# urbste/OpenImuCameraCalibrator

Measured on AMD Instinct MI355X. Metric: residual+Jacobian blocks/sec; wall-clock per LM iter, GoPro9 full calib, higher is better.
Workload: dtype f64

## Files before the change

### openimucameracalibrator_amd/csrc/kernels_bcr.hip

```cpp
#include <hip/hip_runtime.h>
#include <mutex>
#include <unordered_map>
#include "oicc_device.h"
#include "lm_decide.h"
#include "lm_launch.h"
#include "lm_retract.h"
#include "../../include/oicc_hip.h"

namespace oicc {


struct BcrArgs {
  double* D;
  double* F;
  double* S;
  double* Lf;
  double* Mc;
  double* x;
  int32_t* fail;
  long long* prof;
  int n, a, Pb, rtf, LD;
  int delay;
  int o, s, p, m, pn;
  int64_t offS_in, offS_out;
  int carry;
  int last;
  int side;
  int top_l, top_r;
  int b0, ghost;
  const LmCtl* ctl;
};
#define BCR_RETURN_IF_DONE(A) do { if ((A).ctl != nullptr && (A).ctl->done != 0) return; } while (0)

__device__ __forceinline__ void bcr_lds_barrier() { asm volatile("s_waitcnt lgkmcnt(0)\n\ts_barrier" ::: "memory"); }
__device__ __forceinline__ double bcr_readlane(double v, int lane) {
  const int lo = __builtin_amdgcn_readlane(__double2loint(v), lane);
  const int hi = __builtin_amdgcn_readlane(__double2hiint(v), lane);
  return __hiloint2double(hi, lo);
}
typedef double bcr_v4d __attribute__((ext_vector_type(4)));

__device__ __forceinline__ void tri10(int t, int& xt, int& yt) {
  xt = t < 1 ? 0 : (t < 3 ? 1 : (t < 6 ? 2 : 3));
  yt = t - (xt * (xt + 1)) / 2;
}

template <int LD>
__device__ __forceinline__ void bcr_corner_solve(double* C, double* da, int* failp, int a, int tid, int wave, int lane) {
  const int a1 = a + 1;
  if (a1 <= 16) {
    if (wave == 0) {
      double av[16], dinv = 0.0;
#pragma unroll
      for (int c = 0; c < 16; ++c) av[c] = (c < a && lane < a1 && lane >= c) ? C[c * LD + lane] : 0.0;
      bool bad = false;
#pragma unroll
      for (int c = 0; c < 16; ++c) {
        if (c < a) {
          const double piv = bcr_readlane(av[c], c);
          bad |= !(piv > 0.0);
          const double y0 = __builtin_amdgcn_rsq(piv);
          const double g0 = piv * y0, h0 = 0.5 * y0;
          const double r0 = fma(-g0, h0, 0.5);
// ... 63 lines not shown
constexpr int kBackWaves = 8;
constexpr int kInvWaves = 16;
constexpr int kInvLD = 145;

template <int XT>
__device__ __forceinline__ bcr_v4d bcri_z_tile(const double* W, int yt, int li, int lq) {
  constexpr int LD = kInvLD, K0 = 4 * XT, NK = 16 - K0;
  const double* py = W + lq * LD + 64 + 16 * yt + li;
  const double* px = W + lq * LD + 64 + 16 * XT + li;
  double vy[NK], vx[NK];
#pragma unroll
  for (int kk = 0; kk < NK; ++kk) { vy[kk] = py[4 * (K0 + kk) * LD]; vx[kk] = px[4 * (K0 + kk) * LD]; }
  asm volatile("" ::: "memory");
  bcr_v4d g = {0.0, 0.0, 0.0, 0.0}, g2 = {0.0, 0.0, 0.0, 0.0};
#pragma unroll
  for (int kk = 0; kk < NK; kk += 2) {
    g = __builtin_amdgcn_mfma_f64_16x16x4f64(vy[kk], vx[kk], g, 0, 0, 0);
    g2 = __builtin_amdgcn_mfma_f64_16x16x4f64(vy[kk + 1], vx[kk + 1], g2, 0, 0, 0);
  }
  g += g2;
  return g;
}

template <bool LAST>
__device__ __forceinline__ void bcri_tail(const BcrArgs& A, double* W, double* da, int* failp, const double* Fs, double* Zg, int tid, int wave, int lane, bool report,
                                          const double (&ttop)[16], const double ytop, double* x0s) {
  constexpr int LD = kInvLD, NW = kInvWaves, NT = 64 * NW, FLD = 65;
  const int li = lane & 15, lq = lane >> 4;
  const int a = A.a, a1 = a + 1;
  for (int t = wave; t < 10; t += NW) {
    int xt, yt; tri10(t, xt, yt);
    const bcr_v4d g = xt == 0 ? bcri_z_tile<0>(W, yt, li, lq) : (xt == 1 ? bcri_z_tile<1>(W, yt, li, lq) : (xt == 2 ? bcri_z_tile<2>(W, yt, li, lq) : bcri_z_tile<3>(W, yt, li, lq)));
#pragma unroll
    for (int r = 0; r < 4; ++r) {
      const int x = 16 * xt + li, y = 16 * yt + lq + 4 * r;
      if (LAST) { W[y * LD + x] = g[r]; if (xt != yt) W[x * LD + y] = g[r]; }
      else { Zg[y * 64 + x] = g[r]; if (xt != yt) Zg[x * 64 + y] = g[r]; }
    }
  }
  __syncthreads();
  if (!LAST) {
    if (report && tid == 0 && *failp) atomicOr(A.fail, 1);
    return;
  }
  const int rtf = A.rtf;
  if (wave < 4 * rtf) {
    const int t = wave >> 2, w = wave & 3;
    const double* pf = Fs + lq * FLD + 16 * t + li;
    const double* pz = W + lq * LD + 16 * w + li;
    double vf[16], vz[16];
#pragma unroll
    for (int kk = 0; kk < 16; ++kk) { vf[kk] = pf[4 * kk * FLD]; vz[kk] = pz[4 * kk * LD]; }
    asm volatile("" ::: "memory");
    bcr_v4d tq = {0.0, 0.0, 0.0, 0.0};
#pragma unroll
    for (int kk = 0; kk < 16; ++kk) tq = __builtin_amdgcn_mfma_f64_16x16x4f64(vf[kk], vz[kk], tq, 0, 0, 0);
#pragma unroll
    for (int r = 0; r < 4; ++r) W[(16 * w + li) * LD + 64 + 16 * t + lq + 4 * r] = tq[r];
  }
  __syncthreads();
  if (wave < (rtf * (rtf + 1)) / 2) {
    int t1 = 0, u = wave; while (u >= t1 + 1) { u -= t1 + 1; ++t1; }
    const int t2 = u;
    const double* pt = W + lq * LD + 64 + 16 * t1 + li;
    const double* pf = Fs + lq * FLD + 16 * t2 + li;
    double vt[16], vf[16];
#pragma unroll
    for (int kk = 0; kk < 16; ++kk) { vt[kk] = pt[4 * kk * LD]; vf[kk] = pf[4 * kk * FLD]; }
    asm volatile("" ::: "memory");
    bcr_v4d g = {0.0, 0.0, 0.0, 0.0};
#pragma unroll
    for (int kk = 0; kk < 16; ++kk) g = __builtin_amdgcn_mfma_f64_16x16x4f64(vf[kk], vt[kk], g, 0, 0, 0);
    const double* Sm = A.side != 0 ? A.Lf + (int64_t)A.last * (192 + a1) * 64 + 4096 + 64 * a1 : nullptr;
    double mc[4];
#pragma unroll
    for (int r = 0; r < 4; ++r) { const int q1 = 16 * t1 + li, q2 = 16 * t2 + lq + 4 * r; mc[r] = (q1 < a1 && q2 < a1) ? A.Mc[q1 * a1 + q2] + (Sm != nullptr ? Sm[q1 * a1 + q2] : 0.0) : 0.0; }
#pragma unroll
    for (int r = 0; r < 4; ++r) { const int q1 = 16 * t1 + li, q2 = 16 * t2 + lq + 4 * r; if (q1 < a1 && q2 < a1) W[q2 * LD + q1] = mc[r] - g[r]; }
  }
  __syncthreads();
  bcr_corner_solve<LD>(W, da, failp, a, tid, wave, lane);
  for (int q = tid; q < a; q += NT) A.x[A.Pb + q] = da[q];
  if (wave == 0) {
    const double* tc = W + lane * LD + 64;
    double v = tc[a];
    for (int q = 0; q < a; q += 8) {
      double t8[8], d8[8];
#pragma unroll
      for (int k = 0; k < 8; ++k) { const bool ok = q + k < a; t8[k] = ok ? tc[q + k] : 0.0; d8[k] = ok ? da[q + k] : 0.0; }
#pragma unroll
      for (int k = 0; k < 8; ++k) v = fma(-t8[k], d8[k], v);
    }
    const int gi = A.last * 64 + lane;
    if (gi < A.Pb) A.x[gi] = v;
    x0s[lane] = gi < A.Pb ? v : 0.0;
  }
  __syncthreads();
  if (tid == 0 && *failp) atomicOr(A.fail, 1);
  if (A.top_l >= 0 || A.top_r >= 0) {
    double sum_r = 0.0, sum_l = 0.0;
#pragma unroll
    for (int k = 0; k < 4; ++k) {
      const int r = wave + NW * k;
      const double xn = x0s[r], xa = r < a ? da[r] : 0.0;
      sum_r = fma(ttop[k], xn, sum_r);     sum_r = fma(ttop[4 + k], xa, sum_r);
      sum_l = fma(ttop[8 + k], xn, sum_l); sum_l = fma(ttop[12 + k], xa, sum_l);
    }
    W[wave * 64 + lane] = sum_r;
    W[(NW + wave) * 64 + lane] = sum_l;
    __syncthreads();
    if (wave < 2) {
      const int blk = wave == 0 ? A.top_r : A.top_l;
      double acc = 0.0;
#pragma unroll
      for (int w = 0; w < NW; ++w) acc += W[(wave * NW + w) * 64 + lane];
      const int gi = blk * 64 + lane;
      if (blk >= 0 && gi < A.Pb) A.x[gi] = ytop - acc;
    }
  }
}


template <bool LAST, bool PROF, class LoadD>
__device__ __forceinline__ void bcri_invert_body(const BcrArgs& A, const int i, LoadD load_d, const bool report = true) {
  constexpr int LD = kInvLD, NW = kInvWaves, NT = 64 * NW, NTILE = 20, SLOTS = (NTILE + NW - 1) / NW, RU = 128, NAW = 3, FLD = 65;
  static_assert(NW == 16, "the corner phases of block 0 take one tile per wave");
  extern __shared__ double lds[];
  const int tid = threadIdx.x, lane = tid & 63;
  const int wave = __builtin_amdgcn_readfirstlane(tid >> 6);
  const int li = lane & 15, lq = lane >> 4;
  double* const W = lds;
  double* const da = W + 64 * LD;
  int* const failp = reinterpret_cast<int*>(da + 64);
  double* const dg = da + 64 + 8;
  double* const Fs = dg + 256;
  const int a1 = A.a + 1;
  double* Zg = A.Lf + (int64_t)i * (192 + a1) * 64;
  const double* Fg = A.F + (int64_t)i * 64 * a1;
  const double* Sf = (LAST && A.side != 0) ? Zg + 4096 : nullptr;
  const bool prof = PROF && A.prof != nullptr && blockIdx.x == 0 && wave == 0;
  long long pc[8] = {0, 0, 0, 0, 0, 0, 0, 0};
  long long tprev = prof ? clock64() : 0;
// ... 97 lines not shown
#pragma unroll
      for (int k = 0; k < SLOTS; ++k) {
        if (t_ok[k] && t_ct[k] > p && (t_rt[k] < 4 || t_rt[k] - 4 <= p)) {
          const double* pa = W + (j0 + lq) * LD + 16 * t_ct[k] + li;
          const double* pb = W + (j0 + lq) * LD + 16 * t_rt[k] + li;
          double va[4], vb[4];
#pragma unroll
          for (int kq = 0; kq < 4; ++kq) { va[kq] = pa[4 * kq * LD]; vb[kq] = -pb[4 * kq * LD]; }
#pragma unroll
          for (int kq = 0; kq < 4; ++kq) acc[k] = __builtin_amdgcn_mfma_f64_16x16x4f64(va[kq], vb[kq], acc[k], 0, 0, 0);
          if (t_ct[k] == p + 1) {
            double* dst = W + (16 * t_ct[k] + lq) * LD + 16 * t_rt[k] + li;
            dst[0] = acc[k][0]; dst[4 * LD] = acc[k][1]; dst[8 * LD] = acc[k][2]; dst[12 * LD] = acc[k][3];
            if (t_rt[k] == t_ct[k]) { dg[lq * 16 + li] = acc[k][0]; dg[(lq + 4) * 16 + li] = acc[k][1]; dg[(lq + 8) * 16 + li] = acc[k][2]; dg[(lq + 12) * 16 + li] = acc[k][3]; }
          }
        }
      }
    }
    BCR_MARK(3);
    bcr_lds_barrier();
    BCR_MARK(4);
  }
  BCR_MARK(4);
  bcri_tail<LAST>(A, W, da, failp, Fs, Zg, tid, wave, lane, report, ttop, ytop, dg);
  BCR_MARK(5);
  if (PROF && prof && lane == 0) for (int k = 0; k < 8; ++k) A.prof[k] = pc[k];
#undef BCR_MARK
}

template <bool LAST, bool PROF>
__global__ __launch_bounds__(64 * kInvWaves) void bcri_invert_kernel(BcrArgs A) {
  BCR_RETURN_IF_DONE(A);
  const int i = LAST ? A.last : A.o + A.s * (2 * (int)blockIdx.x + A.p);
  const double* Dg = A.D + (int64_t)i * 4096;
  const double* Sd = (LAST && A.side != 0) ? A.Lf + (int64_t)i * (192 + A.a + 1) * 64 : nullptr;
  bcri_invert_body<LAST, PROF>(A, i, [Dg, Sd](int e) { double v = Dg[e]; if (LAST && Sd != nullptr && (e & 63) >= (e >> 6)) v += Sd[e]; return v; });
}

__global__ __launch_bounds__(256) void bcri_schur_kernel(BcrArgs A) {
  BCR_RETURN_IF_DONE(A);
  __shared__ double Ts[16][68];
  const int tid = threadIdx.x, lane = tid & 63;
  const int wave = __builtin_amdgcn_readfirstlane(tid >> 6);
  const int li = lane & 15, lq = lane >> 4;
  const int a1 = A.a + 1, rtf = A.rtf, s = A.s;
  if ((int)blockIdx.y == (int)gridDim.y - 1 && A.carry > 0) {
    const int m = A.carry;
    const double* src = A.S + (A.offS_in + (m - 1)) * 4096; double* dst = A.S + (A.offS_out + (m - 1) / 2) * 4096;
    for (int e = (int)blockIdx.x * 256 + tid; e < 4096; e += (int)gridDim.x * 256) dst[e] = src[e];
// ... 87 lines not shown
      const int x = 16 * xt + li, y = 16 * yt + lq + 4 * r;
      if (to_side) { if (x >= y) Sd[y * 64 + x] = v; }
      else if (x >= y && v != 0.0) unsafeAtomicAdd((xk == 0 ? Dl : Dr) + y * 64 + x, v);
    } else if (yk < 2) {
      const int q = 16 * xt + li, y = 16 * yt + lq + 4 * r;
      if (to_side) { if (q < a1) Sd[4096 + y * a1 + q] = v; }
      else if (q < a1 && v != 0.0) unsafeAtomicAdd((yk == 0 ? Fl : Fr) + y * a1 + q, v);
    } else {
      const int q1 = 16 * xt + li, q2 = 16 * yt + lq + 4 * r;
      if (to_side) { if (q1 < a1 && q2 <= q1) { Sd[4096 + 64 * a1 + q1 * a1 + q2] = v; Sd[4096 + 64 * a1 + q2 * a1 + q1] = v; } }
      else if (q1 < a1 && q2 <= q1 && v != 0.0) {
        unsafeAtomicAdd(A.Mc + q1 * a1 + q2, v);
        if (q1 != q2) unsafeAtomicAdd(A.Mc + q2 * a1 + q1, v);
      }
    }
  }
}

struct BcrOwn {
  int e = -1, code = -1;
  double sc0 = 0.0, d2 = 0.0, g = 0.0;
  const double* x = nullptr; double* xc = nullptr;
};
constexpr int kRetractPark = 12;
template <int NB>
__device__ __forceinline__ BcrOwn bcr_retract_claim(const BcrArgs& A, const RetractReq& R, const SolveBuffers& sb, int b_lo, int b_hi, bool arrow_wg, int tid) {
  BcrOwn o; o.x = R.x; o.xc = R.xc;
  NormalEq ne = R.ne;
  if (A.ctl != nullptr) { o.x = A.ctl->xp[0]; o.xc = A.ctl->xp[1]; ne.base = A.ctl->nep[0]; }
  const int e_hi = b_hi * 64 < A.Pb ? b_hi * 64 : A.Pb;
  if (tid < 64 * NB) { const int e = b_lo * 64 + tid; if (e < e_hi) o.e = e; }
  else if (tid < 64 * NB + A.a && arrow_wg) o.e = A.Pb + (tid - 64 * NB);
  if (o.e >= 0) { o.code = R.rmap[o.e]; o.sc0 = sb.scale[o.e]; o.d2 = sb.D2[o.e]; o.g = ne.g()[o.e]; }
  return o;
}
__device__ __forceinline__ int bcr_rm_steps(int kind) { return kind == kRmEucl ? 1 : (kind == kRmTic ? 6 : 3); }
__device__ __forceinline__ int bcr_rm_params(int kind) { return kind == kRmEucl ? 1 : (kind == kRmTic ? 7 : (kind == kRmSo3 || kind == kRmPt ? 4 : 3)); }
__device__ __forceinline__ void bcr_retract_park(const SolveBuffers& sb, const BcrOwn& o, double* rpark, int stride, int tid) {
  if (o.code < 0) return;
  const int kind = o.code & 7; const int64_t po = o.code >> 3;
  const int nd = bcr_rm_steps(kind), np = bcr_rm_params(kind);
  for (int c = 0; c < np; ++c) rpark[c * stride + tid] = o.x[po + c];
  for (int c = 1; c < nd; ++c) rpark[(6 + c) * stride + tid] = sb.scale[o.e + c];
}
template <int OW>
__device__ __forceinline__ void bcr_retract_finish(const BcrArgs& A, const RetractReq& R, const SolveBuffers& sb, const BcrOwn& o, const double* xflat, int e_base,
                                                   const double* xarrow, const double* rpark, int stride, double* red, int tid, int wave, int lane) {
  __syncthreads();
  if (blockIdx.x == 0 && tid == 0) {
    if (A.ctl != nullptr) { if (A.ctl->stamps != nullptr && A.ctl->seq < A.ctl->trace_cap) A.ctl->stamps[3 * A.ctl->seq + 1] = wall_clock64(); }
    else *R.ne.cost() = 0.0;
  }
  double step_sq = 0.0, x_sq = 0.0, model = 0.0;
  if (o.e >= 0) {
    auto step_at = [&](int e) { return e >= A.Pb ? xarrow[e - A.Pb] : xflat[e - e_base]; };
    model = lm_model_term(step_at(o.e), o.d2, o.g, o.sc0);
    if (o.code >= 0) {
      const int kind = o.code & 7;
      const double alpha = R.alpha;
      const int nd = bcr_rm_steps(kind), np = bcr_rm_params(kind);
      double d[6], sc[6], pv[7];
#pragma unroll
      for (int c = 0; c < 6; ++c) { d[c] = c < nd ? step_at(o.e + c) : 0.0; sc[c] = c == 0 ? o.sc0 : (c < nd ? rpark[(6 + c) * stride + tid] : 0.0); }
#pragma unroll
      for (int c = 0; c < 7; ++c) pv[c] = c < np ? rpark[c * stride + tid] : 0.0;
      double* out = o.xc + (o.code >> 3);
      if (kind == kRmSo3) lm_store_so3(lm_retract_so3(Quat{pv[0], pv[1], pv[2], pv[3]}, d, sc, alpha), pv, out, step_sq, x_sq);
      else if (kind == kRmEucl) lm_retract_eucl(pv[0], d[0], sc[0], alpha, out, step_sq, x_sq);
      else if (kind == kRmAb || kind == kRmGb) { const double bound = kind == kRmAb ? R.max_ab : R.max_gb; for (int c = 0; c < 3; ++c) lm_retract_box(pv[c], d[c], sc[c], alpha, bound, out + c, step_sq, x_sq); }
      else if (kind == kRmPt) lm_retract_point(pv, d, sc, alpha, out, step_sq, x_sq);
      else if (kind == kRmTic) lm_retract_tic(pv, d, sc, alpha, out, step_sq, x_sq);
    }
  }
  if (wave < OW) {
#pragma unroll
    for (int off = 32; off > 0; off >>= 1) { step_sq += __shfl_xor(step_sq, off); x_sq += __shfl_xor(x_sq, off); model += __shfl_xor(model, off); }
    if (lane == 0) { red[wave] = step_sq; red[64 + wave] = x_sq; red[128 + wave] = model; }
  }
  __syncthreads();
  if (tid < 3) {
    double acc = 0.0;
    for (int w = 0; w < OW; ++w) acc += red[64 * tid + w];
    unsafeAtomicAdd(tid == 0 ? &sb.st->step_norm_sq : (tid == 1 ? &sb.st->x_norm_sq : &sb.st->model_cost_change), acc);
  }
}

__global__ __launch_bounds__(64 * kBackWaves) void bcri_backward_kernel(BcrArgs A) {
  BCR_RETURN_IF_DONE(A);
  __shared__ double xs[192];
  __shared__ double part[kBackWaves][64];
  const int tid = threadIdx.x, lane = tid & 63;
  const int wave = __builtin_amdgcn_readfirstlane(tid >> 6);
  const int a = A.a, a1 = a + 1, s = A.s;
  const int kp = 2 * (int)blockIdx.x + A.p;
  const int i = A.o + kp * s, il = i - s;
  const bool hasL = kp > 0;
  const bool hasR = kp < A.m - 1 || A.ghost != 0;
  const int ir = kp < A.m - 1 ? i + s : A.n;
  const double* Tg = A.Lf + (int64_t)i * (192 + a1) * 64 + 4096;
  constexpr int RW = 192 / kBackWaves;
  double lv[RW];
#pragma unroll
  for (int k = 0; k < RW; ++k) {
    const int r = wave + kBackWaves * k;
    const bool ok = r < 128 + a && (hasL || r >= 64) && (hasR || r < 64 || r >= 128);
    lv[k] = ok ? Tg[r * 64 + lane] : 0.0;
  }
  const double yv = wave == 0 ? Tg[(128 + a) * 64 + lane] : 0.0;
  double xin = 0.0;
  if (tid < 64) { const int gi = il * 64 + tid; xin = (hasL && gi < A.Pb) ? A.x[gi] : 0.0; }
  else if (tid < 128) { const int gi = ir * 64 + (tid - 64); xin = (hasR && gi < A.Pb) ? A.x[gi] : 0.0; }
  else if (tid < 128 + a) xin = A.x[A.Pb + (tid - 128)];
  if (tid < 192) xs[tid] = xin;
  __syncthreads();
  double sum = 0.0;
#pragma unroll
  for (int k = 0; k < RW; ++k) { const int r = wave + kBackWaves * k; sum = fma(lv[k], r < 128 + a ? xs[r] : 0.0, sum); }
  part[wave][lane] = sum;
  __syncthreads();
  if (wave == 0) {
    double acc = 0.0;
#pragma unroll
    for (int w = 0; w < kBackWaves; ++w) acc += part[w][lane];
    const int gi = i * 64 + lane;
    if (gi < A.Pb) A.x[gi] = yv - acc;
  }
}

template <bool RETRACT>
__device__ __forceinline__ void bcri_backward2_body(const BcrArgs& A, int ou, int pu, int mu, int npiv_upper, int orphan_l, int orphan_r, const RetractReq& R, const SolveBuffers& sb) {
  constexpr int NW = 16, RW1 = 192 / NW, RW2 = 192 / (NW / 2);
  __shared__ double xw[6][64];
  __shared__ double part[NW][64];
  double* const xs0 = xw[0]; double* const xs1 = xw[2]; double* const xs2 = xw[4]; double* const xs3 = xw[5];
  const int tid = threadIdx.x, lane = tid & 63;
  const int wave = __builtin_amdgcn_readfirstlane(tid >> 6);
  const int a = A.a, a1 = a + 1, s = A.s, n = A.n;
  const int64_t ru64 = (int64_t)(192 + a1) * 64;
  const int lone_ix = (int)blockIdx.x - npiv_upper;
  const bool lone = lone_ix >= 0;
  const bool lone_l = lone && orphan_l >= 0 && lone_ix == 0, lone_r = lone && !lone_l;
  const int ku = 2 * (int)blockIdx.x + pu;
  const int j = lone_l ? orphan_l - s : (lone_r ? orphan_r + s : ou + ku * 2 * s);
  const int jl = j - 2 * s, jr = j + 2 * s;
  const bool ghost = A.ghost != 0;
  const bool has_jl = lone_r || (!lone && ku > 0);
  const bool has_jr = lone_l || (!lone && (ku < mu - 1 || ghost));
  const int jrs = (!lone && ku == mu - 1) ? n : jr;
  const int half = wave >> 3, hw = wave & 7;
  const int ci = half == 0 ? j - s : j + s;
  const bool child = lone ? (half == 0 ? lone_r : lone_l) : (half == 0 ? ci >= A.o : ci <= A.o + (A.m - 1) * s);
  const bool child_hasL = half == 0 ? has_jl : !lone;
  const bool child_hasR = half == 0 ? (!lone || ghost) : has_jr;
  auto xin = [&](int blk, int r) { const int gi = blk * 64 + r; return gi < A.Pb ? A.x[gi] : 0.0; };
  if (tid < 64) xs0[tid] = has_jl ? xin(jl, tid) : 0.0;
  else if (tid < 128) xs2[tid - 64] = has_jr ? xin(jrs, tid - 64) : 0.0;
  else if (tid < 192) xs3[tid - 128] = tid - 128 < a ? A.x[A.Pb + (tid - 128)] : 0.0;
  else if (tid < 256 && lone) xs1[tid - 192] = (lone_r && ghost) ? xin(n, tid - 192) : 0.0;
  __shared__ double rpark[RETRACT ? kRetractPark : 1][384];
  BcrOwn own;
  if (RETRACT) {
    const int b_lo = j - 2 > 0 ? j - 2 : 0;
    int b_hi = j + 2 < n ? j + 2 : n;
    if (!lone && (int)blockIdx.x == npiv_upper - 1 && orphan_r < 0) b_hi = n;
    own = bcr_retract_claim<5>(A, R, sb, b_lo, b_hi, blockIdx.x == 0, tid);
  }
  double l1[RW1], l2[RW2], y1 = 0.0, y2 = 0.0;
  {
    const double* T1 = A.Lf + (lone ? 0 : j) * ru64 + 4096;
#pragma unroll
    for (int k = 0; k < RW1; ++k) {
      const int r = wave + NW * k;
      const bool ok = !lone && r < 128 + a && (has_jl || r >= 64) && (has_jr || r < 64 || r >= 128);
      l1[k] = ok ? T1[r * 64 + lane] : 0.0;
    }
    if (wave == 0 && !lone) y1 = T1[(128 + a) * 64 + lane];
    const double* T2 = A.Lf + (child ? ci : 0) * ru64 + 4096;
#pragma unroll
    for (int k = 0; k < RW2; ++k) {
      const int r = hw + 8 * k;
      const bool ok = child && r < 128 + a && (child_hasL || r >= 64) && (child_hasR || r < 64 || r >= 128);
      l2[k] = ok ? T2[r * 64 + lane] : 0.0;
    }
    if (hw == 0 && child) y2 = T2[(128 + a) * 64 + lane];
  }
  if (RETRACT) bcr_retract_park(sb, own, &rpark[0][0], 384, tid);
  __syncthreads();
  if (!lone) {
    double sum = 0.0;
#pragma unroll
    for (int k = 0; k < RW1; ++k) {
      const int r = wave + NW * k;
      const double xv = r < 64 ? xs0[r] : (r < 128 ? xs2[r - 64] : (r < 128 + a ? xs3[r - 128] : 0.0));
      sum = fma(l1[k], xv, sum);
    }
    part[wave][lane] = sum;
    __syncthreads();
    if (wave == 0) {
      double acc = 0.0;
#pragma unroll
      for (int w = 0; w < NW; ++w) acc += part[w][lane];
      const double xv = y1 - acc;
      const int gi = j * 64 + lane;
      xs1[lane] = gi < A.Pb ? xv : 0.0;
      if (gi < A.Pb) A.x[gi] = xv;
    }
    __syncthreads();
  }
  {
    const double* xl = half == 0 ? xs0 : xs1;
    const double* xr = half == 0 ? xs1 : xs2;
    double sum = 0.0;
#pragma unroll
    for (int k = 0; k < RW2; ++k) {
      const int r = hw + 8 * k;
      const double xv = r < 64 ? xl[r] : (r < 128 ? xr[r - 64] : (r < 128 + a ? xs3[r - 128] : 0.0));
      sum = fma(l2[k], xv, sum);
    }
    part[wave][lane] = sum;
    __syncthreads();
    if (hw == 0 && child) {
      double acc = 0.0;
#pragma unroll
      for (int w = 0; w < 8; ++w) acc += part[8 * half + w][lane];
      const int gi = ci * 64 + lane;
      const double xv = y2 - acc;
      if (gi < A.Pb) A.x[gi] = xv;
      if (RETRACT) xw[half == 0 ? 1 : 3][lane] = gi < A.Pb ? xv : 0.0;
    }
  }
  if (RETRACT) bcr_retract_finish<6>(A, R, sb, own, &xw[0][0], (j - 2) * 64, xs3, &rpark[0][0], 384, &part[0][0], tid, wave, lane);
}
__global__ __launch_bounds__(1024) void bcri_backward2_kernel(BcrArgs A, int ou, int pu, int mu, int npiv_upper, int orphan_l, int orphan_r) {
  BCR_RETURN_IF_DONE(A);
  bcri_backward2_body<false>(A, ou, pu, mu, npiv_upper, orphan_l, orphan_r, RetractReq{}, SolveBuffers{});
}
__global__ __launch_bounds__(1024) void bcri_backward2_retract_kernel(BcrArgs A, int ou, int pu, int mu, int npiv_upper, int orphan_l, int orphan_r, RetractReq R, SolveBuffers sb) {
  BCR_RETURN_IF_DONE(A);
  bcri_backward2_body<true>(A, ou, pu, mu, npiv_upper, orphan_l, orphan_r, R, sb);
}

__device__ __forceinline__ void bcr_build_body(const NormalEq& ne, const TangentLayout& tl, const SolveBuffers& sb, int reuse_diagonal, double min_diag,
                                               double max_diag, const BcrArgs& A, const int64_t tid, const int64_t nthreads) {
  const int Pb = tl.Pb, a = tl.a, W = tl.W, a1 = a + 1, hb = tl.hb, n = A.n;
  const int64_t r0 = (int64_t)A.b0 * 64;
  const double radius = sb.radius;
  if (tid == 0) {
    sb.st->radius = radius; sb.st->model_cost_change = 0.0; sb.st->step_norm_sq = 0.0; sb.st->x_norm_sq = 0.0; sb.st->cand_cost = 0.0; sb.st->chol_failed = 0;
    if (sb.ctl != nullptr && sb.ctl->stamps != nullptr && sb.ctl->seq < sb.ctl->trace_cap) sb.ctl->stamps[3 * sb.ctl->seq] = wall_clock64();
  }
  auto damp = [&](int64_t i, double hii) -> double {
    const double sc = sb.scale[i];
    return (reuse_diagonal ? sb.diag[i] : fmin(fmax(hii * sc * sc, min_diag), max_diag)) / radius;
  };
  for (int64_t i = tid; i < tl.P; i += nthreads) {
    const double hii = i < Pb ? ne.band()[i * W] : ne.C()[(i - Pb) * a + (i - Pb)];
    const double sc = sb.scale[i];
    double d;
    if (!reuse_diagonal) { d = fmin(fmax(hii * sc * sc, min_diag), max_diag); sb.diag[i] = d; }
    else d = sb.diag[i];
    sb.D2[i] = d / radius;
  }
// ... 162 lines not shown
  const int g = A.ghost != 0 ? 1 : 0;
  for (int l = 0; l < L.nlev; ++l) {
    const int m = L.active[l], npiv = L.npivs[l];
    bcr_set_level(A, L, l);
    A.side = (l == L.nlev - 1 && L.parity[l] == 0) ? 1 : 0;
    const bool carry = g != 0 && (m & 1) != 0;
    A.carry = carry ? m : 0;
    BcrArgs Ai = A; if (l != 0) Ai.prof = nullptr;
    if (!(level0_inverted && l == 0)) hipLaunchKernelGGL(k_inv, dim3(npiv), dim3(64 * kInvWaves), bcr_lds_inv(), st, Ai);
    hipLaunchKernelGGL(bcri_schur_kernel, dim3(12 + 3 * A.rtf, npiv + (carry ? 1 : 0)), dim3(256), 0, st, A);
  }
}
static bool bcr_launch_back(BcrArgs A, const BcrLevels& L, int top, hipStream_t st, const RetractReq* R = nullptr, const SolveBuffers* sb = nullptr) {
  int l = top;
  bool fused = false;
  if (l >= 0 && !(l & 1)) { bcr_set_level(A, L, l); hipLaunchKernelGGL(bcri_backward_kernel, dim3(L.npivs[l]), dim3(64 * kBackWaves), 0, st, A); --l; }
  for (; l >= 1; l -= 2) {
    const int lo = l - 1;
    const int orphan_l = (L.parity[lo] == 0 && L.parity[l] == 1) ? L.origin[lo] : -1;
    const int orphan_r = (((L.active[lo] - 1) & 1) == L.parity[lo] && ((L.active[l] - 1) & 1) != L.parity[l]) ? L.origin[lo] + (L.active[lo] - 1) * L.strides[lo] : -1;
    bcr_set_level(A, L, lo);
    const dim3 grid(L.npivs[l] + (orphan_l >= 0 ? 1 : 0) + (orphan_r >= 0 ? 1 : 0));
    if (lo == 0 && R != nullptr) {
      hipLaunchKernelGGL(bcri_backward2_retract_kernel, grid, dim3(1024), 0, st, A, L.origin[l], L.parity[l], L.active[l], L.npivs[l], orphan_l, orphan_r, *R, *sb);
      fused = true;
    } else hipLaunchKernelGGL(bcri_backward2_kernel, grid, dim3(1024), 0, st, A, L.origin[l], L.parity[l], L.active[l], L.npivs[l], orphan_l, orphan_r);
  }
  return fused;
}
static bool bcr_launch_last_and_back(BcrArgs A, const BcrLevels& L, hipStream_t st, const RetractReq* R = nullptr, const SolveBuffers* sb = nullptr) {
  using KernelFn = void (*)(BcrArgs);
  KernelFn k_inv_last = bcri_invert_kernel<true, false>;
  const size_t lds_inv_last = bcr_lds_inv() + (size_t)64 * 65 * sizeof(double);
  bcr_allow_lds(reinterpret_cast<const void*>(k_inv_last), lds_inv_last);
  const int nlev = L.nlev;
  A.o = 0; A.s = 0; A.p = 1; A.m = 1; A.pn = 1; A.offS_in = 0; A.offS_out = 0; A.carry = 0;
  A.last = L.last; A.top_l = -1; A.top_r = -1; A.side = (nlev >= 1 && L.parity[nlev - 1] == 0) ? 1 : 0;
  if (nlev >= 1) {
    const int t = nlev - 1;
    A.top_r = L.last + L.strides[t];
    if (L.parity[t] == 0) A.top_l = L.last - L.strides[t];
  }
  hipLaunchKernelGGL(k_inv_last, dim3(1), dim3(64 * kInvWaves), lds_inv_last, st, A);
  return bcr_launch_back(A, L, nlev - 2, st, R, sb);
}

int bcr_route(const TangentLayout& tl, const SolveBuffers& sb) {
  if (!bcr_applicable(tl) || tl.a + 1 > sb.bcr_max_border || sb.ws == nullptr || sb.ws_doubles < bcr_workspace_doubles(tl)) return kRouteNone;
  if (sb.algo != 0 && sb.algo != 4) return kRouteNone;
  return bcr_fused_build(bcr_blocks(tl.Pb), sb.prof) ? kRouteBcrFused : kRouteBcrUnfused;
}
int launch_bcr_solve(const NormalEq& ne, const TangentLayout& tl, const SolveBuffers& sb, int reuse_diagonal,
                     double min_diag, double max_diag, hipStream_t st, const RetractReq* retract, bool* fused) {
  if (fused) *fused = false;
  if (bcr_route(tl, sb) == kRouteNone) return -1;
  const int n = bcr_blocks(tl.Pb), a1 = tl.a + 1;
  BcrArgs A{};
  bcr_carve(A, sb.ws, n, a1);
  A.Mc = sb.Mc; A.x = sb.step_s; A.fail = &sb.st->chol_failed; A.prof = sb.prof;
  A.n = n; A.a = tl.a; A.Pb = tl.Pb; A.delay = sb.bcr_delay;
  A.rtf = (a1 + 15) / 16; A.ctl = sb.ctl;
  const BcrLevels L = bcr_plan(n, 0, false);
  const bool inverted = bcr_launch_build(ne, tl, sb, reuse_diagonal, min_diag, max_diag, A, L, st);
  bcr_launch_forward(A, inverted, L, st);
  const bool honour = retract != nullptr && retract->on != 0 && retract->rmap != nullptr && retract->alpha == 1.0 && L.nlev >= 3 && A.ghost == 0 && A.b0 == 0;
  RetractReq R{}; if (honour) { R = *retract; R.ne = ne; }
  const bool did = bcr_launch_last_and_back(A, L, st, honour ? &R : nullptr, &sb);
  if (fused) *fused = did;
  return 0;
}

__global__ void bcr_dist_pack_kernel(BcrArgs A, int64_t off_final, double* msg) {
  const int a1 = A.a + 1; const int64_t fsz = (int64_t)64 * a1;
  const int64_t total = 3 * 4096 + 2 * fsz + (int64_t)a1 * a1;
  for (int64_t e = (int64_t)blockIdx.x * blockDim.x + threadIdx.x; e < total; e += (int64_t)gridDim.x * blockDim.x) {
    double v;
    if (e < 4096) v = A.D[e];
    else if (e < 4096 + fsz) v = A.F[e - 4096];
    else if (e < 2 * 4096 + fsz) v = A.ghost ? A.S[off_final * 4096 + (e - 4096 - fsz)] : 0.0;
    else if (e < 3 * 4096 + fsz) v = A.ghost ? A.D[(int64_t)A.n * 4096 + (e - 2 * 4096 - fsz)] : 0.0;
    else if (e < 3 * 4096 + 2 * fsz) v = A.ghost ? A.F[(int64_t)A.n * fsz + (e - 3 * 4096 - fsz)] : 0.0;
    else v = A.Mc[e - 3 * 4096 - 2 * fsz];
    msg[e] = v;
  }
}
__global__ void bcr_dist_top_kernel(BcrArgs T, const double* msgs, int64_t piece) {
  const int N = T.n, a1 = T.a + 1; const int64_t fsz = (int64_t)64 * a1;
  const int64_t nD = (int64_t)N * 4096, nF = (int64_t)N * fsz, nS = (int64_t)(N - 1) * 4096, nC = (int64_t)a1 * a1;
// ... 113 lines not shown
```

### openimucameracalibrator_amd/csrc/oicc_problem.hip

```cpp
#include "oicc_problem.h"

namespace oicc {

int eval_pass(oicc_problem* p, const PassRequest& rq) {
  const double* const x = rq.x; const bool jac = rq.jac; const int only_kind = rq.only_kind;
  const oicc_allreduce_fn reduce = rq.local ? nullptr : p->reduce;
  hipStream_t st = p->stream;
  const NormalEq ne = rq.target ? *rq.target : p->ne;
  if (p->opt["debug_poison_lds"] != 0.0) launch_lds_poison(st);
  {
    const bool with_points = jac && p->tl.a_pts > 0 && (only_kind < 0 || only_kind == 0);
    if (jac && (p->tp.direct || p->tp.n_tiles == 0)) HIPCK(p, hipMemsetAsync(ne.base, 0, ne.total * sizeof(double), st));
    else if (jac && p->tl.a_pts > 0) {
      const int a_np = p->tl.a - p->tl.a_pts;
      HIPCK(p, hipMemsetAsync(ne.base + ne.off_E + int64_t(a_np) * p->tl.Pb, 0, size_t(ne.off_g - ne.off_E - int64_t(a_np) * p->tl.Pb) * sizeof(double), st));
      HIPCK(p, hipMemsetAsync(ne.g() + p->tl.Pb + a_np, 0, size_t(p->tl.a_pts) * sizeof(double), st));
    }
    else if (!jac && !rq.cost_already_zero) HIPCK(p, hipMemsetAsync(ne.cost(), 0, sizeof(double), st));
    const TileParams& tp = p->tp;
    const bool gmax_folded = jac && rq.gmax_into != nullptr && !tp.direct && tp.n_tiles > 0 && !reduce && p->tl.a_pts == 0;
    if (rq.gmax_folded) *rq.gmax_folded = gmax_folded;
    if (!p->h_tstatic) { p->h_tstatic.reset(new TileStatic); std::memset(p->h_tstatic.get(), 0, sizeof(TileStatic)); p->tstatic_valid = false; }
    {
      static_assert(std::is_trivially_copyable<TileStatic>::value, "TileStatic is copied bytewise");
// ... 892 lines not shown
  float ms = 0; (void)hipEventElapsedTime(&ms, ev.a, ev.b);
  if (ms_per_solve) *ms_per_solve = double(ms) / std::max(repeats, 1);
  return OICC_OK;
}

int oicc_solve_residual(oicc_problem* p, int32_t flags, double radius, double out[3]) {
  int rc = prepare(p, flags); if (rc) return rc;
  SolveBuffers sb = solve_buffers(p);
  rc = system_at_current_point(p, local_pass(p->d_x.p, true), sb.scale, p->opt["jacobi_scaling"] != 0, 0.0); if (rc) return rc;
  if (p->tl.P == 0) { out[0] = out[1] = out[2] = 0.0; return OICC_OK; }
  if (launch_lm_solve(p->ne, p->tl, sb, radius, 0, p->opt["min_lm_diagonal"], p->opt["max_lm_diagonal"], p->stream) != 0) { p->err = "solver geometry unsupported"; return OICC_ERR_UNSUPPORTED; }
  return read_solve_residual(p, sb, &out[0], &out[1], &out[2]);
}



double oicc_debug_ls_next_step_size(const double init[3], const double* prev, int32_t prev_has_slope, const double cur[3], int32_t cur_has_slope) {
  LsSample i, q, c;
  i.x = init[0]; i.value = init[1]; i.gradient = init[2]; i.has_gradient = true;
  c.x = cur[0]; c.value = cur[1]; c.gradient = cur[2]; c.has_gradient = cur_has_slope != 0;
  if (prev) { q.x = prev[0]; q.value = prev[1]; q.gradient = prev[2]; q.has_gradient = prev_has_slope != 0; }
  return ls_next_step_size(i, prev ? &q : nullptr, c);
}
int oicc_debug_solver_profile(oicc_problem* p, int32_t flags, long long out[12]) {
  int rc = prepare(p, flags); if (rc) return rc;
  hipStream_t st = p->stream;
  const TangentLayout& tl = p->tl;
  DevBuf<long long> d; if (!d.resize(12)) return OICC_ERR_HIP;
  SolveBuffers sb = solve_buffers(p, d.p);
  rc = system_at_current_point(p, full_system_pass(p), sb.scale, true, 1e4); if (rc) return rc;
  for (int rep = 0; rep < 2; ++rep) {
    if (launch_lm_solve(p->ne, tl, sb, 1e4, 0, 1e-6, 1e32, st) != 0) return OICC_ERR_UNSUPPORTED;
  }
  HIPCK(p, hipMemcpyAsync(out, d.p, 12 * sizeof(long long), hipMemcpyDeviceToHost, st));
  HIPCK(p, hipStreamSynchronize(st));
  return OICC_OK;
}

static int tile_profile(oicc_problem* p, int32_t flags, int32_t kind, long long* out, int n_out) {
  int rc = prepare(p, flags); if (rc) return rc;
  DevBuf<long long> d; if (!d.resize(16)) return OICC_ERR_HIP;
  HIPCK(p, hipMemsetAsync(d.p, 0, 16 * sizeof(long long), p->stream));
  PassRequest rq = local_pass(p->d_x.p, true, kind); rq.prof = d.p;
  rc = eval_pass(p, rq); if (rc) return rc;
  HIPCK(p, hipMemcpyAsync(out, d.p, size_t(n_out) * sizeof(long long), hipMemcpyDeviceToHost, p->stream));
  HIPCK(p, hipStreamSynchronize(p->stream));
  return OICC_OK;
}
int oicc_debug_tile_profile(oicc_problem* p, int32_t flags, int32_t kind, long long out[16]) { return tile_profile(p, flags, kind, out, 16); }
int oicc_debug_block_profile(oicc_problem* p, int32_t flags, int32_t kind, long long out[4]) { return tile_profile(p, flags, kind % 10, out, 4); }
int oicc_debug_view_profile(oicc_problem* p, int32_t flags, long long out[4]) { return oicc_debug_block_profile(p, flags, 0, out); }

int oicc_get_T_i_c(const oicc_problem* p, double v[7]) { std::memcpy(v, p->x.data() + p->pl.tic, 7 * sizeof(double)); return OICC_OK; }
int oicc_get_gravity(const oicc_problem* p, double g[3]) { std::memcpy(g, p->x.data() + p->pl.g, 3 * sizeof(double)); return OICC_OK; }
int oicc_get_rs_line_delay(const oicc_problem* p, double* s) { *s = p->x[p->pl.ld]; return OICC_OK; }
int oicc_get_imu_intrinsics(const oicc_problem* p, double a[6], double g[9]) {
  std::memcpy(a, p->x.data() + p->pl.ai, 6 * sizeof(double)); std::memcpy(g, p->x.data() + p->pl.gi, 9 * sizeof(double)); return OICC_OK; }
int64_t oicc_get_num_accl_bias_knots(const oicc_problem* p) { return p->pl.n_ab; }
int64_t oicc_get_num_gyro_bias_knots(const oicc_problem* p) { return p->pl.n_gb; }
int oicc_get_bias_knots(const oicc_problem* p, double* a, int64_t na, double* g, int64_t ng) {
// ... 60 lines not shown
```

Before: 50.75 million.

## Move arrow retraction into a dedicated block and prefetch retract parameters early

The fused backward-substitution and retraction kernel now gives the arrow (global parameter) retraction its own extra workgroup. Before, those threads were claimed inside block 0's retraction, so that block carried the extra work. Retraction parameter loads are issued into registers before the first barrier and written to LDS after the partial sums, shrinking the LDS park buffer from 12 to 6 rows and overlapping global loads with compute. The fused path is skipped when the tic block lives in the block-tridiagonal part. Profiling timers are also added to the last inversion tail, plus a new debug entry point.

```diff
diff --git a/openimucameracalibrator_amd/csrc/kernels_bcr.hip b/openimucameracalibrator_amd/csrc/kernels_bcr.hip
--- a/openimucameracalibrator_amd/csrc/kernels_bcr.hip
+++ b/openimucameracalibrator_amd/csrc/kernels_bcr.hip
@@ -39,6 +39,8 @@
   return __hiloint2double(hi, lo);
 }
 typedef double bcr_v4d __attribute__((ext_vector_type(4)));
+typedef const __attribute__((address_space(1))) double* bcr_gptr;
+__device__ __forceinline__ bcr_gptr bcr_global(const double* p) { return (bcr_gptr)p; }
 
 __device__ __forceinline__ void tri10(int t, int& xt, int& yt) {
   xt = t < 1 ? 0 : (t < 3 ? 1 : (t < 6 ? 2 : 3));
@@ -148,12 +150,14 @@
   return g;
 }
 
-template <bool LAST>
+template <bool LAST, bool PROF>
 __device__ __forceinline__ void bcri_tail(const BcrArgs& A, double* W, double* da, int* failp, const double* Fs, double* Zg, int tid, int wave, int lane, bool report,
-                                          const double (&ttop)[16], const double ytop, double* x0s) {
+                                          const double (&ttop)[16], const double ytop, double* x0s, const bool prof) {
   constexpr int LD = kInvLD, NW = kInvWaves, NT = 64 * NW, FLD = 65;
   const int li = lane & 15, lq = lane >> 4;
   const int a = A.a, a1 = a + 1;
+  long long tprev = (PROF && prof) ? clock64() : 0;
+#define BCR_TMARK(k) do { if (PROF && prof) { const long long tn_ = clock64(); if (lane == 0) A.prof[20 + (k)] = tn_ - tprev; tprev = tn_; } } while (0)
   for (int t = wave; t < 10; t += NW) {
     int xt, yt; tri10(t, xt, yt);
     const bcr_v4d g = xt == 0 ? bcri_z_tile<0>(W, yt, li, lq) : (xt == 1 ? bcri_z_tile<1>(W, yt, li, lq) : (xt == 2 ? bcri_z_tile<2>(W, yt, li, lq) : bcri_z_tile<3>(W, yt, li, lq)));
@@ -165,6 +169,7 @@
     }
   }
   __syncthreads();
+  BCR_TMARK(0);
   if (!LAST) {
     if (report && tid == 0 && *failp) atomicOr(A.fail, 1);
     return;
@@ -185,6 +190,7 @@
     for (int r = 0; r < 4; ++r) W[(16 * w + li) * LD + 64 + 16 * t + lq + 4 * r] = tq[r];
   }
   __syncthreads();
+  BCR_TMARK(1);
   if (wave < (rtf * (rtf + 1)) / 2) {
     int t1 = 0, u = wave; while (u >= t1 + 1) { u -= t1 + 1; ++t1; }
     const int t2 = u;
@@ -205,7 +211,9 @@
     for (int r = 0; r < 4; ++r) { const int q1 = 16 * t1 + li, q2 = 16 * t2 + lq + 4 * r; if (q1 < a1 && q2 < a1) W[q2 * LD + q1] = mc[r] - g[r]; }
   }
   __syncthreads();
+  BCR_TMARK(2);
   bcr_corner_solve<LD>(W, da, failp, a, tid, wave, lane);
+  BCR_TMARK(3);
   for (int q = tid; q < a; q += NT) A.x[A.Pb + q] = da[q];
   if (wave == 0) {
     const double* tc = W + lane * LD + 64;
@@ -222,6 +230,7 @@
     x0s[lane] = gi < A.Pb ? v : 0.0;
   }
   __syncthreads();
+  BCR_TMARK(4);
   if (tid == 0 && *failp) atomicOr(A.fail, 1);
   if (A.top_l >= 0 || A.top_r >= 0) {
     double sum_r = 0.0, sum_l = 0.0;
@@ -244,6 +253,8 @@
       if (blk >= 0 && gi < A.Pb) A.x[gi] = ytop - acc;
     }
   }
+  BCR_TMARK(5);
+#undef BCR_TMARK
 }
 
 
@@ -387,9 +398,9 @@
     BCR_MARK(4);
   }
   BCR_MARK(4);
-  bcri_tail<LAST>(A, W, da, failp, Fs, Zg, tid, wave, lane, report, ttop, ytop, dg);
+  bcri_tail<LAST, PROF>(A, W, da, failp, Fs, Zg, tid, wave, lane, report, ttop, ytop, dg, prof);
   BCR_MARK(5);
-  if (PROF && prof && lane == 0) for (int k = 0; k < 8; ++k) A.prof[k] = pc[k];
+  if (PROF && prof && lane == 0) for (int k = 0; k < 8; ++k) A.prof[(LAST ? 12 : 0) + k] = pc[k];
 #undef BCR_MARK
 }
 
@@ -523,32 +534,50 @@
   double sc0 = 0.0, d2 = 0.0, g = 0.0;
   const double* x = nullptr; double* xc = nullptr;
 };
-constexpr int kRetractPark = 12;
+constexpr int kRetractPark = 6;
 template <int NB>
-__device__ __forceinline__ BcrOwn bcr_retract_claim(const BcrArgs& A, const RetractReq& R, const SolveBuffers& sb, int b_lo, int b_hi, bool arrow_wg, int tid) {
+__device__ __forceinline__ BcrOwn bcr_retract_claim(const BcrArgs& A, const RetractReq& R, const SolveBuffers& sb, int b_lo, int b_hi, int tid) {
   BcrOwn o; o.x = R.x; o.xc = R.xc;
   NormalEq ne = R.ne;
   if (A.ctl != nullptr) { o.x = A.ctl->xp[0]; o.xc = A.ctl->xp[1]; ne.base = A.ctl->nep[0]; }
   const int e_hi = b_hi * 64 < A.Pb ? b_hi * 64 : A.Pb;
   if (tid < 64 * NB) { const int e = b_lo * 64 + tid; if (e < e_hi) o.e = e; }
-  else if (tid < 64 * NB + A.a && arrow_wg) o.e = A.Pb + (tid - 64 * NB);
-  if (o.e >= 0) { o.code = R.rmap[o.e]; o.sc0 = sb.scale[o.e]; o.d2 = sb.D2[o.e]; o.g = ne.g()[o.e]; }
+  if (o.e >= 0) { o.code = R.rmap[o.e]; o.sc0 = sb.scale[o.e]; o.d2 = sb.D2[o.e]; o.g = bcr_global(ne.g())[o.e]; }
   return o;
 }
 __device__ __forceinline__ int bcr_rm_steps(int kind) { return kind == kRmEucl ? 1 : (kind == kRmTic ? 6 : 3); }
 __device__ __forceinline__ int bcr_rm_params(int kind) { return kind == kRmEucl ? 1 : (kind == kRmTic ? 7 : (kind == kRmSo3 || kind == kRmPt ? 4 : 3)); }
-__device__ __forceinline__ void bcr_retract_park(const SolveBuffers& sb, const BcrOwn& o, double* rpark, int stride, int tid) {
+__device__ __forceinline__ void bcr_retract_park_request(const SolveBuffers& sb, const BcrOwn& o, double (&pk)[kRetractPark]) {
+  const int kind = o.code & 7; const int64_t po = o.code >> 3;
+  const int nd = o.code < 0 ? 0 : bcr_rm_steps(kind), np = o.code < 0 ? 0 : bcr_rm_params(kind);
+#pragma unroll
+  for (int c = 0; c < 4; ++c) pk[c] = c < np ? bcr_global(o.x)[po + c] : 0.0;
+#pragma unroll
+  for (int c = 1; c < 3; ++c) pk[3 + c] = c < nd ? sb.scale[o.e + c] : 0.0;
+}
+__device__ __forceinline__ void bcr_retract_park(const BcrOwn& o, const double (&pk)[kRetractPark], double* rpark, int stride, int tid) {
   if (o.code < 0) return;
-  const int kind = o.code & 7; const int64_t po = o.code >> 3;
+  const int kind = o.code & 7;
   const int nd = bcr_rm_steps(kind), np = bcr_rm_params(kind);
-  for (int c = 0; c < np; ++c) rpark[c * stride + tid] = o.x[po + c];
-  for (int c = 1; c < nd; ++c) rpark[(6 + c) * stride + tid] = sb.scale[o.e + c];
+#pragma unroll
+  for (int c = 0; c < 4; ++c) if (c < np) rpark[c * stride + tid] = pk[c];
+#pragma unroll
+  for (int c = 1; c < 3; ++c) if (c < nd) rpark[(3 + c) * stride + tid] = pk[3 + c];
+}
+template <bool TIC>
+__device__ __forceinline__ void bcr_retract_block(const RetractReq& R, int kind, const double (&d)[6], const double (&sc)[6], const double (&pv)[7], double* out, double& step_sq, double& x_sq) {
+  const double alpha = R.alpha;
+  if (kind == kRmSo3) lm_store_so3(lm_retract_so3(Quat{pv[0], pv[1], pv[2], pv[3]}, d, sc, alpha), pv, out, step_sq, x_sq);
+  else if (kind == kRmEucl) lm_retract_eucl(pv[0], d[0], sc[0], alpha, out, step_sq, x_sq);
+  else if (kind == kRmAb || kind == kRmGb) { const double bound = kind == kRmAb ? R.max_ab : R.max_gb; for (int c = 0; c < 3; ++c) lm_retract_box(pv[c], d[c], sc[c], alpha, bound, out + c, step_sq, x_sq); }
+  else if (kind == kRmPt) lm_retract_point(pv, d, sc, alpha, out, step_sq, x_sq);
+  else if (TIC && kind == kRmTic) lm_retract_tic(pv, d, sc, alpha, out, step_sq, x_sq);
 }
 template <int OW>
 __device__ __forceinline__ void bcr_retract_finish(const BcrArgs& A, const RetractReq& R, const SolveBuffers& sb, const BcrOwn& o, const double* xflat, int e_base,
-                                                   const double* xarrow, const double* rpark, int stride, double* red, int tid, int wave, int lane) {
+                                                   const double* xarrow, const double* rpark, int stride, double* red, bool first, int tid, int wave, int lane) {
   __syncthreads();
-  if (blockIdx.x == 0 && tid == 0) {
+  if (first && tid == 0) {
     if (A.ctl != nullptr) { if (A.ctl->stamps != nullptr && A.ctl->seq < A.ctl->trace_cap) A.ctl->stamps[3 * A.ctl->seq + 1] = wall_clock64(); }
     else *R.ne.cost() = 0.0;
   }
@@ -558,19 +587,13 @@
     model = lm_model_term(step_at(o.e), o.d2, o.g, o.sc0);
     if (o.code >= 0) {
       const int kind = o.code & 7;
-      const double alpha = R.alpha;
       const int nd = bcr_rm_steps(kind), np = bcr_rm_params(kind);
       double d[6], sc[6], pv[7];
 #pragma unroll
-      for (int c = 0; c < 6; ++c) { d[c] = c < nd ? step_at(o.e + c) : 0.0; sc[c] = c == 0 ? o.sc0 : (c < nd ? rpark[(6 + c) * stride + tid] : 0.0); }
-#pragma unroll
-      for (int c = 0; c < 7; ++c) pv[c] = c < np ? rpark[c * stride + tid] : 0.0;
-      double* out = o.xc + (o.code >> 3);
-      if (kind == kRmSo3) lm_store_so3(lm_retract_so3(Quat{pv[0], pv[1], pv[2], pv[3]}, d, sc, alpha), pv, out, step_sq, x_sq);
-      else if (kind == kRmEucl) lm_retract_eucl(pv[0], d[0], sc[0], alpha, out, step_sq, x_sq);
-      else if (kind == kRmAb || kind == kRmGb) { const double bound = kind == kRmAb ? R.max_ab : R.max_gb; for (int c = 0; c < 3; ++c) lm_retract_box(pv[c], d[c], sc[c], alpha, bound, out + c, step_sq, x_sq); }
-      else if (kind == kRmPt) lm_retract_point(pv, d, sc, alpha, out, step_sq, x_sq);
-      else if (kind == kRmTic) lm_retract_tic(pv, d, sc, alpha, out, step_sq, x_sq);
+      for (int c = 0; c < 6; ++c) { d[c] = (c < 3 && c < nd) ? step_at(o.e + c) : 0.0; sc[c] = c == 0 ? o.sc0 : ((c < 3 && c < nd) ? rpark[(3 + c) * stride + tid] : 0.0); }
+#pragma unroll
+      for (int c = 0; c < 7; ++c) pv[c] = (c < 4 && c < np) ? rpark[c * stride + tid] : 0.0;
+      bcr_retract_block<false>(R, kind, d, sc, pv, o.xc + (o.code >> 3), step_sq, x_sq);
     }
   }
   if (wave < OW) {
@@ -584,6 +607,37 @@
     for (int w = 0; w < OW; ++w) acc += red[64 * tid + w];
     unsafeAtomicAdd(tid == 0 ? &sb.st->step_norm_sq : (tid == 1 ? &sb.st->x_norm_sq : &sb.st->model_cost_change), acc);
   }
+}
+
+__device__ __forceinline__ void bcr_retract_arrow(const BcrArgs& A, const RetractReq& R, const SolveBuffers& sb) {
+  const int lane = threadIdx.x;
+  if (lane >= 64) return;
+  const int a = A.a;
+  const double* x = R.x; double* xc = R.xc;
+  NormalEq ne = R.ne;
+  if (A.ctl != nullptr) { x = A.ctl->xp[0]; xc = A.ctl->xp[1]; ne.base = A.ctl->nep[0]; }
+  double step_sq = 0.0, x_sq = 0.0, model = 0.0;
+  if (lane < a) {
+    const int e = A.Pb + lane;
+    const int code = R.rmap[e];
+    const double d2 = sb.D2[e], g = bcr_global(ne.g())[e];
+    double d[6], sc[6], pv[7];
+#pragma unroll
+    for (int c = 0; c < 6; ++c) { const bool ok = lane + c < a; d[c] = ok ? A.x[e + c] : 0.0; sc[c] = ok ? sb.scale[e + c] : 0.0; }
+    model = lm_model_term(d[0], d2, g, sc[0]);
+    if (code >= 0) {
+      const int kind = code & 7; const int64_t po = code >> 3;
+      const int nd = bcr_rm_steps(kind), np = bcr_rm_params(kind);
+#pragma unroll
+      for (int c = 0; c < 7; ++c) pv[c] = c < np ? bcr_global(x)[po + c] : 0.0;
+#pragma unroll
+      for (int c = 1; c < 6; ++c) if (c >= nd) { d[c] = 0.0; sc[c] = 0.0; }
+      bcr_retract_block<true>(R, kind, d, sc, pv, xc + po, step_sq, x_sq);
+    }
+  }
+#pragma unroll
+  for (int off = 32; off > 0; off >>= 1) { step_sq += __shfl_xor(step_sq, off); x_sq += __shfl_xor(x_sq, off); model += __shfl_xor(model, off); }
+  if (lane < 3) unsafeAtomicAdd(lane == 0 ? &sb.st->step_norm_sq : (lane == 1 ? &sb.st->x_norm_sq : &sb.st->model_cost_change), lane == 0 ? step_sq : (lane == 1 ? x_sq : model));
 }
 
 __global__ __launch_bounds__(64 * kBackWaves) void bcri_backward_kernel(BcrArgs A) {
@@ -629,7 +683,7 @@
 }
 
 template <bool RETRACT>
-__device__ __forceinline__ void bcri_backward2_body(const BcrArgs& A, int ou, int pu, int mu, int npiv_upper, int orphan_l, int orphan_r, const RetractReq& R, const SolveBuffers& sb) {
+__device__ __forceinline__ void bcri_backward2_body(const BcrArgs& A, const int bx, int ou, int pu, int mu, int npiv_upper, int orphan_l, int orphan_r, const RetractReq& R, const SolveBuffers& sb) {
   constexpr int NW = 16, RW1 = 192 / NW, RW2 = 192 / (NW / 2);
   __shared__ double xw[6][64];
   __shared__ double part[NW][64];
@@ -638,10 +692,10 @@
   const int wave = __builtin_amdgcn_readfirstlane(tid >> 6);
   const int a = A.a, a1 = a + 1, s = A.s, n = A.n;
   const int64_t ru64 = (int64_t)(192 + a1) * 64;
-  const int lone_ix = (int)blockIdx.x - npiv_upper;
+  const int lone_ix = bx - npiv_upper;
   const bool lone = lone_ix >= 0;
   const bool lone_l = lone && orphan_l >= 0 && lone_ix == 0, lone_r = lone && !lone_l;
-  const int ku = 2 * (int)blockIdx.x + pu;
+  const int ku = 2 * bx + pu;
   const int j = lone_l ? orphan_l - s : (lone_r ? orphan_r + s : ou + ku * 2 * s);
   const int jl = j - 2 * s, jr = j + 2 * s;
   const bool ghost = A.ghost != 0;
@@ -654,17 +708,18 @@
   const bool child_hasL = half == 0 ? has_jl : !lone;
   const bool child_hasR = half == 0 ? (!lone || ghost) : has_jr;
   auto xin = [&](int blk, int r) { const int gi = blk * 64 + r; return gi < A.Pb ? A.x[gi] : 0.0; };
-  if (tid < 64) xs0[tid] = has_jl ? xin(jl, tid) : 0.0;
-  else if (tid < 128) xs2[tid - 64] = has_jr ? xin(jrs, tid - 64) : 0.0;
-  else if (tid < 192) xs3[tid - 128] = tid - 128 < a ? A.x[A.Pb + (tid - 128)] : 0.0;
-  else if (tid < 256 && lone) xs1[tid - 192] = (lone_r && ghost) ? xin(n, tid - 192) : 0.0;
-  __shared__ double rpark[RETRACT ? kRetractPark : 1][384];
-  BcrOwn own;
+  double xv0 = 0.0;
+  if (tid < 64) xv0 = has_jl ? xin(jl, tid) : 0.0;
+  else if (tid < 128) xv0 = has_jr ? xin(jrs, tid - 64) : 0.0;
+  else if (tid < 192) xv0 = tid - 128 < a ? A.x[A.Pb + (tid - 128)] : 0.0;
+  else if (tid < 256 && lone) xv0 = (lone_r && ghost) ? xin(n, tid - 192) : 0.0;
+  __shared__ double rpark[RETRACT ? kRetractPark : 1][320];
+  BcrOwn own; double pk[kRetractPark] = {};
   if (RETRACT) {
     const int b_lo = j - 2 > 0 ? j - 2 : 0;
     int b_hi = j + 2 < n ? j + 2 : n;
-    if (!lone && (int)blockIdx.x == npiv_upper - 1 && orphan_r < 0) b_hi = n;
-    own = bcr_retract_claim<5>(A, R, sb, b_lo, b_hi, blockIdx.x == 0, tid);
+    if (!lone && bx == npiv_upper - 1 && orphan_r < 0) b_hi = n;
+    own = bcr_retract_claim<5>(A, R, sb, b_lo, b_hi, tid);
   }
   double l1[RW1], l2[RW2], y1 = 0.0, y2 = 0.0;
   {
@@ -685,7 +740,11 @@
     }
     if (hw == 0 && child) y2 = T2[(128 + a) * 64 + lane];
   }
-  if (RETRACT) bcr_retract_park(sb, own, &rpark[0][0], 384, tid);
+  if (tid < 64) xs0[tid] = xv0;
+  else if (tid < 128) xs2[tid - 64] = xv0;
+  else if (tid < 192) xs3[tid - 128] = xv0;
+  else if (tid < 256 && lone) xs1[tid - 192] = xv0;
+  if (RETRACT) bcr_retract_park_request(sb, own, pk);
   __syncthreads();
   if (!lone) {
     double sum = 0.0;
@@ -696,6 +755,9 @@
       sum = fma(l1[k], xv, sum);
     }
     part[wave][lane] = sum;
+  }
+  if (RETRACT) bcr_retract_park(own, pk, &rpark[0][0], 320, tid);
+  if (!lone) {
     __syncthreads();
     if (wave == 0) {
       double acc = 0.0;
@@ -730,15 +792,16 @@
       if (RETRACT) xw[half == 0 ? 1 : 3][lane] = gi < A.Pb ? xv : 0.0;
     }
   }
-  if (RETRACT) bcr_retract_finish<6>(A, R, sb, own, &xw[0][0], (j - 2) * 64, xs3, &rpark[0][0], 384, &part[0][0], tid, wave, lane);
+  if (RETRACT) bcr_retract_finish<5>(A, R, sb, own, &xw[0][0], (j - 2) * 64, xs3, &rpark[0][0], 320, &part[0][0], bx == 0, tid, wave, lane);
 }
 __global__ __launch_bounds__(1024) void bcri_backward2_kernel(BcrArgs A, int ou, int pu, int mu, int npiv_upper, int orphan_l, int orphan_r) {
   BCR_RETURN_IF_DONE(A);
-  bcri_backward2_body<false>(A, ou, pu, mu, npiv_upper, orphan_l, orphan_r, RetractReq{}, SolveBuffers{});
+  bcri_backward2_body<false>(A, (int)blockIdx.x, ou, pu, mu, npiv_upper, orphan_l, orphan_r, RetractReq{}, SolveBuffers{});
 }
 __global__ __launch_bounds__(1024) void bcri_backward2_retract_kernel(BcrArgs A, int ou, int pu, int mu, int npiv_upper, int orphan_l, int orphan_r, RetractReq R, SolveBuffers sb) {
   BCR_RETURN_IF_DONE(A);
-  bcri_backward2_body<true>(A, ou, pu, mu, npiv_upper, orphan_l, orphan_r, R, sb);
+  if (blockIdx.x == 0) { bcr_retract_arrow(A, R, sb); return; }
+  bcri_backward2_body<true>(A, (int)blockIdx.x - 1, ou, pu, mu, npiv_upper, orphan_l, orphan_r, R, sb);
 }
 
 __device__ __forceinline__ void bcr_build_body(const NormalEq& ne, const TangentLayout& tl, const SolveBuffers& sb, int reuse_diagonal, double min_diag,
@@ -947,7 +1010,7 @@
     bcr_set_level(A, L, lo);
     const dim3 grid(L.npivs[l] + (orphan_l >= 0 ? 1 : 0) + (orphan_r >= 0 ? 1 : 0));
     if (lo == 0 && R != nullptr) {
-      hipLaunchKernelGGL(bcri_backward2_retract_kernel, grid, dim3(1024), 0, st, A, L.origin[l], L.parity[l], L.active[l], L.npivs[l], orphan_l, orphan_r, *R, *sb);
+      hipLaunchKernelGGL(bcri_backward2_retract_kernel, dim3(grid.x + 1), dim3(1024), 0, st, A, L.origin[l], L.parity[l], L.active[l], L.npivs[l], orphan_l, orphan_r, *R, *sb);
       fused = true;
     } else hipLaunchKernelGGL(bcri_backward2_kernel, grid, dim3(1024), 0, st, A, L.origin[l], L.parity[l], L.active[l], L.npivs[l], orphan_l, orphan_r);
   }
@@ -955,7 +1018,7 @@
 }
 static bool bcr_launch_last_and_back(BcrArgs A, const BcrLevels& L, hipStream_t st, const RetractReq* R = nullptr, const SolveBuffers* sb = nullptr) {
   using KernelFn = void (*)(BcrArgs);
-  KernelFn k_inv_last = bcri_invert_kernel<true, false>;
+  KernelFn k_inv_last = A.prof ? bcri_invert_kernel<true, true> : bcri_invert_kernel<true, false>;
   const size_t lds_inv_last = bcr_lds_inv() + (size_t)64 * 65 * sizeof(double);
   bcr_allow_lds(reinterpret_cast<const void*>(k_inv_last), lds_inv_last);
   const int nlev = L.nlev;
@@ -988,7 +1051,8 @@
   const BcrLevels L = bcr_plan(n, 0, false);
   const bool inverted = bcr_launch_build(ne, tl, sb, reuse_diagonal, min_diag, max_diag, A, L, st);
   bcr_launch_forward(A, inverted, L, st);
-  const bool honour = retract != nullptr && retract->on != 0 && retract->rmap != nullptr && retract->alpha == 1.0 && L.nlev >= 3 && A.ghost == 0 && A.b0 == 0;
+  const bool honour = retract != nullptr && retract->on != 0 && retract->rmap != nullptr && retract->alpha == 1.0 && L.nlev >= 3 && A.ghost == 0 && A.b0 == 0 &&
+                      (tl.tic < 0 || tl.tic >= tl.Pb);
   RetractReq R{}; if (honour) { R = *retract; R.ne = ne; }
   const bool did = bcr_launch_last_and_back(A, L, st, honour ? &R : nullptr, &sb);
   if (fused) *fused = did;
diff --git a/openimucameracalibrator_amd/csrc/oicc_problem.hip b/openimucameracalibrator_amd/csrc/oicc_problem.hip
--- a/openimucameracalibrator_amd/csrc/oicc_problem.hip
+++ b/openimucameracalibrator_amd/csrc/oicc_problem.hip
@@ -938,20 +938,24 @@
   if (prev) { q.x = prev[0]; q.value = prev[1]; q.gradient = prev[2]; q.has_gradient = prev_has_slope != 0; }
   return ls_next_step_size(i, prev ? &q : nullptr, c);
 }
-int oicc_debug_solver_profile(oicc_problem* p, int32_t flags, long long out[12]) {
+static int solver_profile(oicc_problem* p, int32_t flags, long long out[12], long long* tail) {
   int rc = prepare(p, flags); if (rc) return rc;
   hipStream_t st = p->stream;
   const TangentLayout& tl = p->tl;
-  DevBuf<long long> d; if (!d.resize(12)) return OICC_ERR_HIP;
+  DevBuf<long long> d; if (!d.resize(32)) return OICC_ERR_HIP;
+  HIPCK(p, hipMemsetAsync(d.p, 0, 32 * sizeof(long long), st));
   SolveBuffers sb = solve_buffers(p, d.p);
   rc = system_at_current_point(p, full_system_pass(p), sb.scale, true, 1e4); if (rc) return rc;
   for (int rep = 0; rep < 2; ++rep) {
     if (launch_lm_solve(p->ne, tl, sb, 1e4, 0, 1e-6, 1e32, st) != 0) return OICC_ERR_UNSUPPORTED;
   }
   HIPCK(p, hipMemcpyAsync(out, d.p, 12 * sizeof(long long), hipMemcpyDeviceToHost, st));
+  if (tail) HIPCK(p, hipMemcpyAsync(tail, d.p + 12, 14 * sizeof(long long), hipMemcpyDeviceToHost, st));
   HIPCK(p, hipStreamSynchronize(st));
   return OICC_OK;
 }
+int oicc_debug_solver_profile(oicc_problem* p, int32_t flags, long long out[12]) { return solver_profile(p, flags, out, nullptr); }
+int oicc_debug_solver_tail_profile(oicc_problem* p, int32_t flags, long long out[14]) { long long head[12]; return solver_profile(p, flags, head, out); }
 
 static int tile_profile(oicc_problem* p, int32_t flags, int32_t kind, long long* out, int n_out) {
   int rc = prepare(p, flags); if (rc) return rc;
```

New measurement: 50.74 million. No clear change (-0.0%).
